# neel-dey/anatomix

Hardware: AMD Instinct MI355X
Metric: 128^3 volumes/sec feature-extraction (6M UNet) (higher is better)
Workload: dtype f16; 1 GPU; anatomix 6M UNet (ngf=16,num_downs=4) forward on sw_batch=4 windows of 1x128^3 (the predictor call of sliding_window_inference, BASELINE configs[1] / the metric); fp32 NCDHW in/out, 16-bit (f16) channels-last activations, fp32 accumulate; holds the 1e-3 tolerance against the fp32 reference in rel-L2 ONLY (max-norm 0.86e-3 .. 1.4e-3 by weight seed; the mode that holds both norms is value_strict); batch_per_gpu=4, window=128, parallelism=replicas x1 (no data-path collective)

## Files before the change

anatomix_amd/csrc/amx_conv3d_upmerge.hip:

```cpp
#include <stdio.h>
#include <stdlib.h>

#include "amx_device.h"

namespace amx {


template <int Q, int TZ, int TY, int NBUF, int KS, bool SPLIT = false, int LXT = 16>
struct UpmCfg {
  static_assert(LXT == 16 || LXT == 8, "a tile is 16 cells of one low-res row, or 8 cells of two rows (rows shorter than 16)");
  static constexpr int RPT = 16 / LXT;
  static constexpr int BY = TY * RPT;
  static constexpr int NP = SPLIT ? 2 : 1;
  static_assert(!SPLIT || KS == 1, "strict precision: 32-channel stages");
  static constexpr int T = TZ * TY;
  static constexpr int HZ = TZ + 2, HY = BY + 2, HX = LXT + 2, HV = HZ * HY * HX;
  static constexpr int PL = ((HV * 16 + 255) / 256) * 256;
  static constexpr int BUF = 4 * KS * NP * PL;
  static constexpr int NJ = (HV + 63) / 64;
  static constexpr int NDMA = 4 * KS * NP * NJ;
  static constexpr int PER_WAVE = (NDMA + 7) / 8;
  static constexpr int LDS_BYTES = NBUF * BUF;
  static_assert(LDS_BYTES <= 160 * 1024, "ring must fit the LDS");
};

template <typename T_, int Q, int TZ, int TY, int NBUF, int KS, bool SPLIT, int LXT>
__global__ __launch_bounds__(512) void conv3d_upmerge_kernel(const UpmergeParams p) {
  typedef UpmCfg<Q, TZ, TY, NBUF, KS, SPLIT, LXT> C;
  constexpr int RPT = C::RPT, BY = C::BY;
  constexpr int NP = C::NP;
  typedef typename Ops<T_>::vec8 vec8;
  constexpr int HY = C::HY, HX = C::HX, PL = C::PL, NT = C::T;
  extern __shared__ __attribute__((aligned(16))) char smem[];

  const int tid = threadIdx.x, lane = tid & 63;
  const int wave = __builtin_amdgcn_readfirstlane(tid >> 6);
  const int li = lane & 15, g = lane >> 4;
  const int lix = li & (LXT - 1), liy = LXT == 8 ? li >> 3 : 0;
  const int pz = wave >> 2, py = (wave >> 1) & 1, px = wave & 1;

  const int nbricks = p.nbz * p.nby * p.nbx * p.N;
  const int ncg = p.Cout / (16 * Q);
  const int items = nbricks * ncg;
  const int G = gridDim.x;
  int jw = blockIdx.x;
  if ((G & 7) == 0) jw = (jw & 7) * (G >> 3) + (jw >> 3);
  const int it0 = (int)((long long)items * jw / G), it1 = (int)((long long)items * (jw + 1) / G);
  const int nstage = p.C1 / (32 * KS);
  const int T_total = (it1 - it0) * nstage;
  if (T_total <= 0) return;

  struct Item { int bx, by, bz, n, cg; };
  auto decode = [&](int it) {
    Item r;
    r.cg = it / nbricks;
    int b = it - r.cg * nbricks;
    r.bx = b % p.nbx; b /= p.nbx;
    r.by = b % p.nby; b /= p.nby;
    r.bz = b % p.nbz;
    r.n = b / p.nbz;
    return r;
  };

  int dma_item = -1;
  int off[C::PER_WAVE];
  auto issue = [&](int it, int stage, int bsel) {
    const Item I = decode(it);
    if (it != dma_item) {
      dma_item = it;
#pragma unroll
      for (int m = 0; m < C::PER_WAVE; ++m) {
        const int id = wave + 8 * m;
        const int j = id % C::NJ;
        const int hv = j * 64 + lane;
        const int hz = hv / (HY * HX), rem = hv - hz * (HY * HX), hy = rem / HX, hx = rem - hy * HX;
        int gz = I.bz * TZ - 1 + hz, gy = I.by * BY - 1 + hy, gx = I.bx * LXT - 1 + hx;
        gz = gz < 0 ? 0 : (gz >= p.LD ? p.LD - 1 : gz);
        gy = gy < 0 ? 0 : (gy >= p.LH ? p.LH - 1 : gy);
        gx = gx < 0 ? 0 : (gx >= p.LW ? p.LW - 1 : gx);
        off[m] = hv < C::HV ? gz * (int)p.sz + gy * (int)p.sy + gx * (int)p.sx : -1;
      }
    }
    const char* base = p.src + (long long)I.n * p.sn;
    const int cs = p.cs ? p.cs : 32;
    char* buf = smem + bsel * C::BUF;
#pragma unroll
    for (int m = 0; m < C::PER_WAVE; ++m) {
      const int id = wave + 8 * m;
      if (id < C::NDMA) {
        const int plane = id / C::NJ, j = id - plane * C::NJ;
        const int cbyte = stage * (64 * KS) + (SPLIT && plane >= 4 ? p.C1 * 2 + (plane - 4) * 16 : plane * 16);
        if (off[m] >= 0)
          dma16_asm(base + off[m] + (long long)(cbyte >> 5) * cs + (cbyte & 31),
                    (unsigned)__builtin_amdgcn_readfirstlane((int)lds_addr(buf + plane * PL + j * 1024)));
      }
    }
  };

  auto wptr = [&](int it, int stage) -> const char* {
    const int cg = it / nbricks;
    return p.wpk + ((((long long)cg * nstage * KS + stage * KS) * 8 + wave) * 8 * NP * Q) * 1024 + lane * 16;
  };
  auto woff = [](const int e2) { return ((e2 >> 3) * 64 + (e2 & 7)) * NP * Q * 1024; };
  constexpr int NTAP = 8 * KS;
  constexpr int WIN = 4;
  vec8 wq[WIN][NP][Q];
  const int lbase = g * PL + ((pz * HY + py + liy) * HX + px + lix) * 16;

  f32x4 acc[NT][Q];
  int nx_it = it0, nx_stage = 0;
  auto step_next = [&]() {
    if (++nx_stage == nstage) { nx_stage = 0; ++nx_it; }
  };
  issue(nx_it, nx_stage, 0);
  step_next();
  if (NBUF > 2 && T_total > 1) { issue(nx_it, nx_stage, 1); step_next(); }
  {
    const char* w0 = wptr(it0, 0);
#pragma unroll
    for (int e = 0; e < WIN; ++e)
#pragma unroll
      for (int h = 0; h < NP; ++h)
#pragma unroll
        for (int q = 0; q < Q; ++q) wq[e][h][q] = *(const vec8*)(w0 + woff(e) + (h * Q + q) * 1024);
  }

  int cu_it = it0, cu_stage = 0;
  bool bad = false;
  unsigned pend[NT][2 * Q * NP];
  int pend_it = -1;
  unsigned padd[NT][2 * Q * NP];
  auto load_part = [&](const int it) {
    const Item I = decode(it);
    const int lx = I.bx * LXT + lix;
    const int ocs = p.ocs ? p.ocs : 32, cb2 = (I.cg * 16 * Q + g * 4 * Q) * 2;
    const long long sy = (long long)p.Cout * 2 * NP * (2 * p.LW), sz = sy * (2 * p.LH), sx = ocs == 32 ? (long long)p.Cout * 2 * NP : 32;
    const char* pb = p.part + (long long)I.n * sz * (2 * p.LD) + pz * sz + py * sy + (2 * lx + px) * sx + (long long)(cb2 >> 5) * ocs + (cb2 & 31);
#pragma unroll
    for (int i = 0; i < NT; ++i) {
      const int lz = I.bz * TZ + i / TY, ly = I.by * BY + (i % TY) * RPT + liy;
      const bool in = (lz < p.LD) & (ly < p.LH) & (lx < p.LW);
#pragma unroll
      for (int hl = 0; hl < NP; ++hl) {
        const char* src = pb + 2 * lz * sz + 2 * ly * sy + hl * p.Cout * 2;
        unsigned* dst = &padd[i][hl * 2 * Q];
        if (Q == 1) {
          const uint2 v = in ? *(const uint2*)src : make_uint2(0u, 0u);
          dst[0] = v.x; dst[1] = v.y;
        } else {
#pragma unroll
          for (int h = 0; h < Q / 2; ++h) {
            const uint4 v = in ? *(const uint4*)(src + h * 16) : make_uint4(0u, 0u, 0u, 0u);
            dst[4 * h] = v.x; dst[4 * h + 1] = v.y; dst[4 * h + 2] = v.z; dst[4 * h + 3] = v.w;
          }
        }
      }
    }
  };
  auto flush = [&]() {
    const Item I = decode(pend_it);
    pend_it = -1;
    const int lx = I.bx * LXT + lix;
    const int ocs = p.ocs ? p.ocs : 32, cb2 = (I.cg * 16 * Q + g * 4 * Q) * 2;
    const long long sy = (long long)p.Cout * 2 * NP * (2 * p.LW), sz = sy * (2 * p.LH), sx = ocs == 32 ? (long long)p.Cout * 2 * NP : 32;
    char* pb = p.out + (long long)I.n * sz * (2 * p.LD) + pz * sz + py * sy + (2 * lx + px) * sx + (long long)(cb2 >> 5) * ocs + (cb2 & 31);
#pragma unroll
    for (int i = 0; i < NT; ++i) {
      const int lz = I.bz * TZ + i / TY, ly = I.by * BY + (i % TY) * RPT + liy;
      if (lz >= p.LD || ly >= p.LH || lx >= p.LW) continue;
#pragma unroll
      for (int hl = 0; hl < NP; ++hl) {
        char* dst = pb + 2 * lz * sz + 2 * ly * sy + hl * p.Cout * 2;
        const unsigned* v = &pend[i][hl * 2 * Q];
        if (Q == 1) *(uint2*)dst = make_uint2(v[0], v[1]);
        else {
#pragma unroll
          for (int h = 0; h < Q / 2; ++h) *(uint4*)(dst + h * 16) = make_uint4(v[4 * h], v[4 * h + 1], v[4 * h + 2], v[4 * h + 3]);
        }
      }
    }
  };
  for (int t = 0; t < T_total; ++t) {
    if (t == 0) asm volatile("s_waitcnt vmcnt(0)" ::: "memory");
    else asm volatile("" ::"v"(wq[0][0][0]) : "memory");
    __syncthreads();
    if (t + NBUF - 1 < T_total && !(p.dbg & 1)) {
      issue(nx_it, nx_stage, (t + NBUF - 1) % NBUF);
      step_next();
    }
    if (pend_it >= 0 && !(p.dbg & 4)) flush();
    if (cu_stage == nstage - 1 && !(p.dbg & 16)) load_part(cu_it);
    const char* buf = smem + (t % NBUF) * C::BUF + lbase;
    if (cu_stage == 0) {
#pragma unroll
      for (int i = 0; i < NT; ++i)
#pragma unroll
        for (int q = 0; q < Q; ++q) acc[i][q] = f32x4{0.f, 0.f, 0.f, 0.f};
    }
    const bool more = t + 1 < T_total;
    const int w_it = cu_stage + 1 < nstage ? cu_it : cu_it + 1, w_stage = cu_stage + 1 < nstage ? cu_stage + 1 : 0;
    const char* wn = more ? wptr(w_it, w_stage) : p.wpk;
    const char* wc = wptr(cu_it, cu_stage);
    if (!(p.dbg & 2)) {
      constexpr int GT = SPLIT ? 2 : (NT < 4 ? NT : 4), NGT = NT / GT, NG = NTAP * NGT;
      vec8 fb[2][GT][NP];
      auto load_group = [&](const int gi, const int set) {
        const int e2 = gi / NGT, i0 = (gi % NGT) * GT;
        const int ks = e2 >> 3, ez = (e2 >> 2) & 1, ey = (e2 >> 1) & 1, ex = e2 & 1;
#pragma unroll
        for (int k = 0; k < GT; ++k) {
          const int lz = (i0 + k) / TY, ly = (i0 + k) % TY;
#pragma unroll
          for (int h = 0; h < NP; ++h)
            fb[set][k][h] = *(const vec8*)(buf + (ks + h) * 4 * PL + (((lz + ez) * HY + ly * RPT + ey) * HX + ex) * 16);
        }
      };
      load_group(0, 0);
#pragma unroll
      for (int gi = 0; gi < NG; ++gi) {
        const int e = gi / NGT, i0 = (gi % NGT) * GT;
        if (gi + 1 < NG) load_group(gi + 1, (gi + 1) & 1);
        __builtin_amdgcn_sched_barrier(0);
#pragma unroll
        for (int k = 0; k < GT; ++k)
#pragma unroll
          for (int q = 0; q < Q; ++q) {
            acc[i0 + k][q] = Ops<T_>::mfma(wq[e % WIN][0][q], fb[gi & 1][k][0], acc[i0 + k][q]);
            if (SPLIT) {
              acc[i0 + k][q] = Ops<T_>::mfma(wq[e % WIN][0][q], fb[gi & 1][k][NP - 1], acc[i0 + k][q]);
              acc[i0 + k][q] = Ops<T_>::mfma(wq[e % WIN][NP - 1][q], fb[gi & 1][k][0], acc[i0 + k][q]);
            }
          }
        __builtin_amdgcn_sched_barrier(0);
        if ((gi % NGT) == NGT - 1 && (e + WIN < NTAP || more)) {
          const char* src = e + WIN < NTAP ? wc + woff(e + WIN) : wn + woff(e + WIN - NTAP);
#pragma unroll
          for (int h = 0; h < NP; ++h)
#pragma unroll
            for (int q = 0; q < Q; ++q) wq[e % WIN][h][q] = *(const vec8*)(src + (h * Q + q) * 1024);
        }
      }
    }
    if (++cu_stage < nstage) continue;
    cu_stage = 0;

    {
      const int cgb = (cu_it / nbricks) * 16 * Q + g * 4 * Q;
      auto cvt = [](const unsigned w, const int half) { return (float)__builtin_bit_cast(T_, (unsigned short)(half ? w >> 16 : w & 0xffffu)); };
#pragma unroll
      for (int q = 0; q < Q; ++q) {
        const f32x4 bv = p.bias ? *(const f32x4*)(p.bias + cgb + q * 4) : f32x4{0.f, 0.f, 0.f, 0.f};
#pragma unroll
        for (int i = 0; i < NT; ++i)
#pragma unroll
          for (int j = 0; j < 4; ++j) {
            float a = cvt(padd[i][2 * q + (j >> 1)], j & 1);
            if (SPLIT) a += cvt(padd[i][2 * Q + 2 * q + (j >> 1)], j & 1);
            acc[i][q][j] += bv[j] + a;
          }
      }
      act_inplace<NT * Q>(&acc[0][0], p.act, p.slope);
    }
#pragma unroll
    for (int i = 0; i < NT; ++i)
#pragma unroll
      for (int q = 0; q < Q; ++q) {
#pragma unroll
        for (int j = 0; j < 4; ++j)
          if (RangeCheck<T_>::on) bad |= RangeCheck<T_>::bad(acc[i][q][j]);
        pend[i][2 * q] = (unsigned)to_bits<T_>(acc[i][q][0]) | ((unsigned)to_bits<T_>(acc[i][q][1]) << 16);
        pend[i][2 * q + 1] = (unsigned)to_bits<T_>(acc[i][q][2]) | ((unsigned)to_bits<T_>(acc[i][q][3]) << 16);
        if (SPLIT) {
          float r[4];
#pragma unroll
          for (int j = 0; j < 4; ++j) r[j] = acc[i][q][j] - (float)(T_)acc[i][q][j];
          pend[i][2 * Q + 2 * q] = (unsigned)to_bits<T_>(r[0]) | ((unsigned)to_bits<T_>(r[1]) << 16);
          pend[i][2 * Q + 2 * q + 1] = (unsigned)to_bits<T_>(r[2]) | ((unsigned)to_bits<T_>(r[3]) << 16);
        }
      }
    pend_it = cu_it;
    ++cu_it;
  }
  if (pend_it >= 0 && !(p.dbg & 4)) flush();
  if (RangeCheck<T_>::on) raise_flag(p.oflow, bad);
}

template <typename T>
__global__ void pack_upmerge_kernel(const float* __restrict__ w, const float* __restrict__ scale, T* __restrict__ wpk, int c_off,
                                    int CinTotal, int C1, int Cout, int Q, int split) {
  const int nstage = C1 / 32, NP = split ? 2 : 1;
  const long long total = (long long)(Cout / (16 * Q)) * nstage * 64 * NP * Q * 512;
  for (long long idx = blockIdx.x * (long long)blockDim.x + threadIdx.x; idx < total; idx += (long long)gridDim.x * blockDim.x) {
    const int j = idx & 7, lane = (idx >> 3) & 63;
    long long r = idx >> 9;
    const int q = r % Q; r /= Q;
    const int part = r % NP; r /= NP;
    const int e = r % 8; r /= 8;
    const int cls = r % 8; r /= 8;
    const int stage = r % nstage;
    const int cg = (int)(r / nstage);
    const int m = lane & 15, g = lane >> 4;
    const int cout = cg * 16 * Q + (m >> 2) * 4 * Q + q * 4 + (m & 3);
    const int cin = c_off + stage * 32 + g * 8 + j;
    const int par[3] = {cls >> 2, (cls >> 1) & 1, cls & 1};
    const int ee[3] = {e >> 2, (e >> 1) & 1, e & 1};
    int lo[3], hi[3];
    for (int a = 0; a < 3; ++a) {
      if (par[a] == 0) { lo[a] = ee[a] ? 1 : 0; hi[a] = ee[a] ? 2 : 0; }
      else { lo[a] = ee[a] ? 2 : 0; hi[a] = ee[a] ? 2 : 1; }
    }
    float sum = 0.f;
    for (int kz = lo[0]; kz <= hi[0]; ++kz)
      for (int ky = lo[1]; ky <= hi[1]; ++ky)
        for (int kx = lo[2]; kx <= hi[2]; ++kx) sum += w[((long long)cout * CinTotal + cin) * 27 + (kz * 3 + ky) * 3 + kx];
    const float v = sum * (scale ? scale[cout] : 1.f);
    const T vh = (T)v;
    wpk[idx] = part ? (T)(v - (float)vh) : vh;
  }
}

static thread_local char g_kernel_name6[64] = "";
const char* last_conv_upmerge_kernel_name() { return g_kernel_name6; }

size_t conv_upmerge_packed_bytes(int C1, int Cout, int split) { return (size_t)Cout * C1 * 64 * 2 * (split ? 2 : 1); }
size_t conv_upmerge_partial_bytes(int N, int D, int H, int W, int Cout) { return (size_t)N * D * H * W * Cout * 2; }
int conv_upmerge_q(int Cout, int split) { return (!split && Cout % 32 == 0) ? 2 : 1; }

bool conv_upmerge_eligible(int C0, int C1, int Cout, int D, int H, int W, int up_shift, int split) {
  static int off = -1;
  if (off < 0) off = exp_env("AMX_NO_UPMERGE") ? 1 : 0;
  return !off && up_shift == 1 && C0 >= 16 && C1 >= 32 && C1 % 32 == 0 && Cout >= (split ? 16 : 32) && Cout % 16 == 0 && W >= 16 && !(D & 1) && !(H & 1) &&
         !(W & 1) && D >= 4 && H >= 4;
}

static int g_num_cus6 = 0;

template <typename T, int Q, int TZ, int TY, int NBUF, int KS, bool SPLIT = false, int LXT = 16>
static hipError_t launch_upm(UpmergeParams p, hipStream_t st) {
  typedef UpmCfg<Q, TZ, TY, NBUF, KS, SPLIT, LXT> C;
  snprintf(g_kernel_name6, sizeof g_kernel_name6, "conv3d_upmerge<%s,q%d,%dx%dx%d,b%d,k%d>", __is_same(T, f16) ? (SPLIT ? "f16x2" : "f16") : (SPLIT ? "bf16x2" : "bf16"), Q,
           TZ, C::BY, LXT, NBUF, 32 * KS);
  auto kern = conv3d_upmerge_kernel<T, Q, TZ, TY, NBUF, KS, SPLIT, LXT>;
  static amx::DeviceOnce attr_once;
  if (!attr_once.done()) {
    hipError_t e = hipFuncSetAttribute((const void*)kern, hipFuncAttributeMaxDynamicSharedMemorySize, C::LDS_BYTES);
    if (e != hipSuccess) return e;
    attr_once.set();
  }
  if (g_num_cus6 == 0) {
    int dev = 0;
    hipDeviceProp_t prop;
    if (hipGetDevice(&dev) != hipSuccess || hipGetDeviceProperties(&prop, dev) != hipSuccess) return hipErrorUnknown;
    g_num_cus6 = prop.multiProcessorCount > 0 ? prop.multiProcessorCount : 256;
  }
  p.nbz = (p.LD + TZ - 1) / TZ;
  p.nby = (p.LH + C::BY - 1) / C::BY;
  p.nbx = (p.LW + LXT - 1) / LXT;
  static int dbg = -1;
  if (dbg < 0) {
    const char* e = exp_env("AMX_DBG");
    dbg = e ? atoi(e) : 0;
  }
  p.dbg = dbg;
  const long long items = (long long)p.nbz * p.nby * p.nbx * p.N * (p.Cout / (16 * Q));
  const long long grid = items < g_num_cus6 ? items : g_num_cus6;
  hipLaunchKernelGGL(kern, dim3((unsigned)grid), dim3(512), C::LDS_BYTES, st, p);
  return hipGetLastError();
}

template <typename T>
static hipError_t launch_upm_split(const UpmergeParams& p, hipStream_t st) {
  if (p.LW < 16) return launch_upm<T, 1, 2, 2, 3, 1, true, 8>(p, st);
  const long long cells = (long long)p.N * p.LD * p.LH * ((p.LW + 15) / 16);
  if (cells / 8 * (p.Cout / 16) >= 256) return launch_upm<T, 1, 2, 4, 2, 1, true>(p, st);
  return launch_upm<T, 1, 2, 2, 3, 1, true>(p, st);
}

template <typename T>
static hipError_t launch_upm_t(const UpmergeParams& p, hipStream_t st) {
  const int Q = conv_upmerge_q(p.Cout, 0);
  if (p.LW < 16) {
    if (Q == 2) return p.C1 % 64 == 0 ? launch_upm<T, 2, 2, 2, 2, 2, false, 8>(p, st) : launch_upm<T, 2, 2, 2, 3, 1, false, 8>(p, st);
    return launch_upm<T, 1, 2, 2, 3, 1, false, 8>(p, st);
  }
  const long long cells = (long long)p.N * p.LD * p.LH * ((p.LW + 15) / 16);
  const long long groups = p.Cout / (16 * Q);
  const bool k64 = p.C1 % 64 == 0;
  if (Q == 2) {
    if (cells / 8 * groups >= 256) return launch_upm<T, 2, 2, 4, 3, 1>(p, st);
    return k64 ? launch_upm<T, 2, 2, 2, 2, 2>(p, st) : launch_upm<T, 2, 2, 2, 3, 1>(p, st);
  }
  if (cells / 16 * groups >= 256) return launch_upm<T, 1, 2, 8, 3, 1>(p, st);
  return k64 ? launch_upm<T, 1, 2, 4, 2, 2>(p, st) : launch_upm<T, 1, 2, 4, 3, 1>(p, st);
}

hipError_t launch_conv_upmerge(const UpmergeParams& p, int precision, hipStream_t st) {
  if (precision == 0) return launch_upm_t<f16>(p, st);
  if (precision == 1) return launch_upm_t<bf16>(p, st);
  if (precision == 2) return launch_upm_split<f16>(p, st);
  if (precision == 3) return launch_upm_split<bf16>(p, st);
  return hipErrorInvalidValue;
}

hipError_t launch_pack_upmerge(const float* w, const float* scale, void* wpk, int c_off, int CinTotal, int C1, int Cout, int precision,
                               hipStream_t st) {
  const int split = precision >= 2;
  const int Q = conv_upmerge_q(Cout, split);
  const long long total = (long long)Cout * C1 * 64 * (split ? 2 : 1);
  const int blocks = (int)((total + 255) / 256 > 4096 ? 4096 : (total + 255) / 256);
  if ((precision & 1) == 0)
    hipLaunchKernelGGL(pack_upmerge_kernel<f16>, dim3(blocks), dim3(256), 0, st, w, scale, (f16*)wpk, c_off, CinTotal, C1, Cout, Q, split);
  else
    hipLaunchKernelGGL(pack_upmerge_kernel<bf16>, dim3(blocks), dim3(256), 0, st, w, scale, (bf16*)wpk, c_off, CinTotal, C1, Cout, Q, split);
  return hipGetLastError();
}

}
```

Baseline: 2882 volumes/s.

## Split Q=2 channel groups into half-width work items for small 8-wide upmerge

Adds a QH template parameter so a Q=2 packed weight layout can be processed as two Q=1 halves. Each work item then covers half the output channels, which doubles the number of work items when the brick count is too small to fill the CUs. The change also reorders the lane-to-cell mapping for 8-wide tiles and pads the LDS plane size, apparently to reduce LDS bank conflicts. In exchange, each work item reuses its staged input across fewer channels, so input halo traffic per output rises.

```diff
diff --git a/anatomix_amd/csrc/amx_conv3d_upmerge.hip b/anatomix_amd/csrc/amx_conv3d_upmerge.hip
--- a/anatomix_amd/csrc/amx_conv3d_upmerge.hip
+++ b/anatomix_amd/csrc/amx_conv3d_upmerge.hip
@@ -6,7 +6,7 @@
 namespace amx {
 
 
-template <int Q, int TZ, int TY, int NBUF, int KS, bool SPLIT = false, int LXT = 16>
+template <int Q, int TZ, int TY, int NBUF, int KS, bool SPLIT = false, int LXT = 16, int QH = 1>
 struct UpmCfg {
   static_assert(LXT == 16 || LXT == 8, "a tile is 16 cells of one low-res row, or 8 cells of two rows (rows shorter than 16)");
   static constexpr int RPT = 16 / LXT;
@@ -15,7 +15,8 @@
   static_assert(!SPLIT || KS == 1, "strict precision: 32-channel stages");
   static constexpr int T = TZ * TY;
   static constexpr int HZ = TZ + 2, HY = BY + 2, HX = LXT + 2, HV = HZ * HY * HX;
-  static constexpr int PL = ((HV * 16 + 255) / 256) * 256;
+  static constexpr int QP = Q * QH;
+  static constexpr int PL = LXT == 16 ? ((HV * 16 + 255) / 256) * 256 : ((HV * 16 + 127) / 256) * 256 + 128;
   static constexpr int BUF = 4 * KS * NP * PL;
   static constexpr int NJ = (HV + 63) / 64;
   static constexpr int NDMA = 4 * KS * NP * NJ;
@@ -24,11 +25,11 @@
   static_assert(LDS_BYTES <= 160 * 1024, "ring must fit the LDS");
 };
 
-template <typename T_, int Q, int TZ, int TY, int NBUF, int KS, bool SPLIT, int LXT>
+template <typename T_, int Q, int TZ, int TY, int NBUF, int KS, bool SPLIT, int LXT, int QH>
 __global__ __launch_bounds__(512) void conv3d_upmerge_kernel(const UpmergeParams p) {
-  typedef UpmCfg<Q, TZ, TY, NBUF, KS, SPLIT, LXT> C;
+  typedef UpmCfg<Q, TZ, TY, NBUF, KS, SPLIT, LXT, QH> C;
   constexpr int RPT = C::RPT, BY = C::BY;
-  constexpr int NP = C::NP;
+  constexpr int NP = C::NP, QP = C::QP;
   typedef typename Ops<T_>::vec8 vec8;
   constexpr int HY = C::HY, HX = C::HX, PL = C::PL, NT = C::T;
   extern __shared__ __attribute__((aligned(16))) char smem[];
@@ -36,7 +37,8 @@
   const int tid = threadIdx.x, lane = tid & 63;
   const int wave = __builtin_amdgcn_readfirstlane(tid >> 6);
   const int li = lane & 15, g = lane >> 4;
-  const int lix = li & (LXT - 1), liy = LXT == 8 ? li >> 3 : 0;
+  const int cell = LXT == 8 ? (int)((0xDCB7FEA984326510ull >> (4 * li)) & 15) : li;
+  const int lix = cell & (LXT - 1), liy = LXT == 8 ? cell >> 3 : 0;
   const int pz = wave >> 2, py = (wave >> 1) & 1, px = wave & 1;
 
   const int nbricks = p.nbz * p.nby * p.nbx * p.N;
@@ -99,9 +101,10 @@
 
   auto wptr = [&](int it, int stage) -> const char* {
     const int cg = it / nbricks;
-    return p.wpk + ((((long long)cg * nstage * KS + stage * KS) * 8 + wave) * 8 * NP * Q) * 1024 + lane * 16;
-  };
-  auto woff = [](const int e2) { return ((e2 >> 3) * 64 + (e2 & 7)) * NP * Q * 1024; };
+    return p.wpk + ((((long long)(cg / QH) * nstage * KS + stage * KS) * 8 + wave) * 8 * NP * QP + (cg % QH) * Q) * 1024 + lane * 16;
+  };
+  auto woff = [](const int e2) { return ((e2 >> 3) * 64 + (e2 & 7)) * NP * QP * 1024; };
+  auto cout0 = [&](const int cg) { return (cg / QH) * 16 * QP + g * 4 * QP + (cg % QH) * 4 * Q; };
   constexpr int NTAP = 8 * KS;
   constexpr int WIN = 4;
   vec8 wq[WIN][NP][Q];
@@ -122,7 +125,7 @@
 #pragma unroll
       for (int h = 0; h < NP; ++h)
 #pragma unroll
-        for (int q = 0; q < Q; ++q) wq[e][h][q] = *(const vec8*)(w0 + woff(e) + (h * Q + q) * 1024);
+        for (int q = 0; q < Q; ++q) wq[e][h][q] = *(const vec8*)(w0 + woff(e) + (h * QP + q) * 1024);
   }
 
   int cu_it = it0, cu_stage = 0;
@@ -133,7 +136,7 @@
   auto load_part = [&](const int it) {
     const Item I = decode(it);
     const int lx = I.bx * LXT + lix;
-    const int ocs = p.ocs ? p.ocs : 32, cb2 = (I.cg * 16 * Q + g * 4 * Q) * 2;
+    const int ocs = p.ocs ? p.ocs : 32, cb2 = cout0(I.cg) * 2;
     const long long sy = (long long)p.Cout * 2 * NP * (2 * p.LW), sz = sy * (2 * p.LH), sx = ocs == 32 ? (long long)p.Cout * 2 * NP : 32;
     const char* pb = p.part + (long long)I.n * sz * (2 * p.LD) + pz * sz + py * sy + (2 * lx + px) * sx + (long long)(cb2 >> 5) * ocs + (cb2 & 31);
 #pragma unroll
@@ -161,7 +164,7 @@
     const Item I = decode(pend_it);
     pend_it = -1;
     const int lx = I.bx * LXT + lix;
-    const int ocs = p.ocs ? p.ocs : 32, cb2 = (I.cg * 16 * Q + g * 4 * Q) * 2;
+    const int ocs = p.ocs ? p.ocs : 32, cb2 = cout0(I.cg) * 2;
     const long long sy = (long long)p.Cout * 2 * NP * (2 * p.LW), sz = sy * (2 * p.LH), sx = ocs == 32 ? (long long)p.Cout * 2 * NP : 32;
     char* pb = p.out + (long long)I.n * sz * (2 * p.LD) + pz * sz + py * sy + (2 * lx + px) * sx + (long long)(cb2 >> 5) * ocs + (cb2 & 31);
 #pragma unroll
@@ -237,7 +240,7 @@
 #pragma unroll
           for (int h = 0; h < NP; ++h)
 #pragma unroll
-            for (int q = 0; q < Q; ++q) wq[e % WIN][h][q] = *(const vec8*)(src + (h * Q + q) * 1024);
+            for (int q = 0; q < Q; ++q) wq[e % WIN][h][q] = *(const vec8*)(src + (h * QP + q) * 1024);
         }
       }
     }
@@ -245,7 +248,7 @@
     cu_stage = 0;
 
     {
-      const int cgb = (cu_it / nbricks) * 16 * Q + g * 4 * Q;
+      const int cgb = cout0(cu_it / nbricks);
       auto cvt = [](const unsigned w, const int half) { return (float)__builtin_bit_cast(T_, (unsigned short)(half ? w >> 16 : w & 0xffffu)); };
 #pragma unroll
       for (int q = 0; q < Q; ++q) {
@@ -335,12 +338,12 @@
 
 static int g_num_cus6 = 0;
 
-template <typename T, int Q, int TZ, int TY, int NBUF, int KS, bool SPLIT = false, int LXT = 16>
+template <typename T, int Q, int TZ, int TY, int NBUF, int KS, bool SPLIT = false, int LXT = 16, int QH = 1>
 static hipError_t launch_upm(UpmergeParams p, hipStream_t st) {
-  typedef UpmCfg<Q, TZ, TY, NBUF, KS, SPLIT, LXT> C;
-  snprintf(g_kernel_name6, sizeof g_kernel_name6, "conv3d_upmerge<%s,q%d,%dx%dx%d,b%d,k%d>", __is_same(T, f16) ? (SPLIT ? "f16x2" : "f16") : (SPLIT ? "bf16x2" : "bf16"), Q,
-           TZ, C::BY, LXT, NBUF, 32 * KS);
-  auto kern = conv3d_upmerge_kernel<T, Q, TZ, TY, NBUF, KS, SPLIT, LXT>;
+  typedef UpmCfg<Q, TZ, TY, NBUF, KS, SPLIT, LXT, QH> C;
+  snprintf(g_kernel_name6, sizeof g_kernel_name6, "conv3d_upmerge<%s,q%d%s,%dx%dx%d,b%d,k%d>", __is_same(T, f16) ? (SPLIT ? "f16x2" : "f16") : (SPLIT ? "bf16x2" : "bf16"), Q,
+           QH > 1 ? "h2" : "", TZ, C::BY, LXT, NBUF, 32 * KS);
+  auto kern = conv3d_upmerge_kernel<T, Q, TZ, TY, NBUF, KS, SPLIT, LXT, QH>;
   static amx::DeviceOnce attr_once;
   if (!attr_once.done()) {
     hipError_t e = hipFuncSetAttribute((const void*)kern, hipFuncAttributeMaxDynamicSharedMemorySize, C::LDS_BYTES);
@@ -380,6 +383,10 @@
 static hipError_t launch_upm_t(const UpmergeParams& p, hipStream_t st) {
   const int Q = conv_upmerge_q(p.Cout, 0);
   if (p.LW < 16) {
+    static const bool no_qh = exp_env("AMX_UPM_NO_QH") != nullptr;
+    const long long bricks = (long long)p.N * ((p.LD + 1) / 2) * ((p.LH + 3) / 4) * ((p.LW + 7) / 8);
+    if (Q == 2 && !no_qh && bricks * (p.Cout / 32) < 256)
+      return p.C1 % 64 == 0 ? launch_upm<T, 1, 2, 2, 2, 2, false, 8, 2>(p, st) : launch_upm<T, 1, 2, 2, 3, 1, false, 8, 2>(p, st);
     if (Q == 2) return p.C1 % 64 == 0 ? launch_upm<T, 2, 2, 2, 2, 2, false, 8>(p, st) : launch_upm<T, 2, 2, 2, 3, 1, false, 8>(p, st);
     return launch_upm<T, 1, 2, 2, 3, 1, false, 8>(p, st);
   }
```

Result: no change. 2886 volumes/s, median of 6 (+0.1%).
